# uc-vision/taichi-splatting

Hardware: AMD Instinct MI355X
Metric: fwd+bwd Msplats/s (higher is better)
Workload: dtype f32; 1 GPU; config D: 6000000 random 3D gaussians, 2048x2048, SH deg 3, tile 16, fwd+bwd (render_gaussians, loss=image.sum()); n_gaussians=6000000, tile_size=16, sh_degree=3, mode=single, parallelism=single GPU

## Files before the change

taichi_splatting_amd/csrc/mapper.hip:

```cpp
#pragma clang fp contract(off)
#include "common.h"
#include "frame_internal.h"

namespace ms {

__device__ __forceinline__ void load_point7(const float* __restrict__ points, int64_t i, float g[7]) {
#pragma unroll
  for (int k = 0; k < 7; ++k) g[k] = points[i * 7 + k];
}


__device__ __forceinline__ float readlane_f(float v, int lane) {
  return __int_as_float(__builtin_amdgcn_readlane(__float_as_int(v), lane));
}
__device__ __forceinline__ ObbQuery wave_broadcast(const ObbQuery& q, int lane) {
  ObbQuery r;
  r.inv00 = readlane_f(q.inv00, lane); r.inv01 = readlane_f(q.inv01, lane);
  r.inv10 = readlane_f(q.inv10, lane); r.inv11 = readlane_f(q.inv11, lane);
  r.rel_min_x = readlane_f(q.rel_min_x, lane); r.rel_min_y = readlane_f(q.rel_min_y, lane);
  r.min_tile_x = __builtin_amdgcn_readlane(q.min_tile_x, lane); r.min_tile_y = __builtin_amdgcn_readlane(q.min_tile_y, lane);
  r.span_x = __builtin_amdgcn_readlane(q.span_x, lane); r.span_y = __builtin_amdgcn_readlane(q.span_y, lane);
  return r;
}
__device__ __forceinline__ unsigned long long wide_span_lanes(const ObbQuery& q, bool valid, int* my_span) {
  const int span = valid && q.span_x > 0 && q.span_y > 0 ? q.span_x * q.span_y : 0;
  *my_span = span;
  const int total = (int)readlane_f(wave_sum_to_lane63((float)span), 63);
  int thr = total / 32;
  thr = thr > 16 ? thr : 16;
  return __ballot(span > thr);
}
template <typename F>
__device__ __forceinline__ void wave_walk_span(const ObbQuery& b, int tile_size, int row_begin, int row_end, F on_hits) {
  const int n = b.span_x * b.span_y, lane = lane_id();
  for (int base = 0; base < n; base += 64) {
    const int idx = base + lane;
    bool hit = false;
    int tu = 0, tv = 0;
    if (idx < n) {
      tv = idx / b.span_x; tu = idx - tv * b.span_x;
      const int ty = b.min_tile_y + tv;
      hit = ty >= row_begin && ty < row_end && obb_test_tile(b, tu, tv, tile_size);
    }
    on_hits(hit, b.min_tile_x + tu, b.min_tile_y + tv);
  }
}
__device__ __forceinline__ int count_span(const ObbQuery& q, bool valid, int tile_size, int row_begin, int row_end) {
  int span;
  unsigned long long wide = wide_span_lanes(q, valid, &span);
  const bool mine_is_wide = (wide >> lane_id()) & 1ull;
  int count = 0;
  if (span > 0 && !mine_is_wide) {
    for (int tv = 0; tv < q.span_y; ++tv) {
      const int ty = q.min_tile_y + tv;
      if (ty < row_begin || ty >= row_end) continue;
      for (int tu = 0; tu < q.span_x; ++tu)
        if (obb_test_tile(q, tu, tv, tile_size)) ++count;
    }
  }
  while (wide != 0) {
    const int src = __builtin_ctzll(wide);
    wide &= wide - 1;
    const ObbQuery b = wave_broadcast(q, src);
    int total = 0;
    wave_walk_span(b, tile_size, row_begin, row_end, [&](bool hit, int, int) { total += __builtin_popcountll(__ballot(hit)); });
    if (lane_id() == src) count = total;
  }
  return count;
}
template <typename F>
__device__ __forceinline__ void emit_span(const ObbQuery& q, bool valid, int64_t first, int tile_size, int row_begin,
                                          int row_end, F emit) {
  int span;
  unsigned long long wide = wide_span_lanes(q, valid, &span);
  const bool mine_is_wide = (wide >> lane_id()) & 1ull;
  if (span > 0 && !mine_is_wide) {
    int64_t o = first;
    for (int tu = 0; tu < q.span_x; ++tu) {
      for (int tv = 0; tv < q.span_y; ++tv) {
        const int ty = q.min_tile_y + tv;
        if (ty < row_begin || ty >= row_end) continue;
        if (obb_test_tile(q, tu, tv, tile_size)) emit(o++, q.min_tile_x + tu, ty, -1);
      }
    }
  }
  while (wide != 0) {
    const int src = __builtin_ctzll(wide);
    wide &= wide - 1;
    const ObbQuery b = wave_broadcast(q, src);
    const int lo = __builtin_amdgcn_readlane((int)(uint32_t)first, src), hi = __builtin_amdgcn_readlane((int)(uint32_t)(first >> 32), src);
    int64_t o = (int64_t)(((uint64_t)(uint32_t)hi << 32) | (uint32_t)lo);
    wave_walk_span(b, tile_size, row_begin, row_end, [&](bool hit, int tx, int ty) {
      const unsigned long long m = __ballot(hit);
      if (hit) emit(o + (int)__builtin_amdgcn_mbcnt_hi((uint32_t)(m >> 32), __builtin_amdgcn_mbcnt_lo((uint32_t)m, 0u)), tx, ty, src);
      o += __builtin_popcountll(m);
    });
  }
}

__global__ void __launch_bounds__(256)
tile_count_kernel(const float* __restrict__ points, const int32_t* __restrict__ order,
                  const uint32_t* __restrict__ cull_keys, int64_t v, int image_w,
                  int image_h, int tile_size, float alpha_threshold, int row_begin, int row_end,
                  int32_t* __restrict__ counts, float* __restrict__ ordered_points) {
  const int64_t i = (int64_t)blockIdx.x * blockDim.x + threadIdx.x;
  const bool valid = i < v && !(cull_keys && cull_keys[i] == CULLED_DEPTH_KEY);
  float g[7] = {0.f, 0.f, 1.f, 0.f, 1.f, 1.f, 0.f};
  if (valid) {
    load_point7(points, order ? (int64_t)order[i] : i, g);
    if (ordered_points) {
#pragma unroll
      for (int k = 0; k < 7; ++k) ordered_points[i * 7 + k] = g[k];
    }
  }
  const ObbQuery q = obb_grid_query(g, image_w, image_h, tile_size, alpha_threshold);
  const int count = count_span(q, valid, tile_size, row_begin, row_end);
  if (i < v) counts[i] = count;
}

template <typename KeyT, int MODE>
__global__ void __launch_bounds__(256)
tile_emit_kernel(const float* __restrict__ points, const float* __restrict__ depth,
                 const int32_t* __restrict__ order, const int32_t* __restrict__ cum, int64_t v,
                 int image_w, int image_h, int tile_size, float alpha_threshold, int row_begin,
                 int row_end, int points_ordered, const int32_t* __restrict__ k_limit,
                 KeyT* __restrict__ keys, int32_t* __restrict__ values) {
  const int64_t i = (int64_t)blockIdx.x * blockDim.x + threadIdx.x;
  if (k_limit && *k_limit == 0) return;
  const bool valid = i < v && !(k_limit && cum[i + 1] == cum[i]);
  const int64_t src = valid ? (order ? (int64_t)order[i] : i) : 0;
  float g[7] = {0.f, 0.f, 1.f, 0.f, 1.f, 1.f, 0.f};
  if (valid) load_point7(points, points_ordered ? i : src, g);
  const ObbQuery q = obb_grid_query(g, image_w, image_h, tile_size, alpha_threshold);
  const int tiles_wide = image_w / tile_size;
  KeyT depth_key = 0;
  if (valid) {
    if (MODE == 1) {
      const float c = fminf(fmaxf(depth[src], 0.0f), 1.0f);
      depth_key = (KeyT)(uint32_t)(c * 65535.0f);
    } else if (MODE == 0) {
      depth_key = (KeyT)__float_as_uint(depth[src]);
    }
  }
  const uint32_t dk_lo = (uint32_t)depth_key, dk_hi = (uint32_t)((uint64_t)depth_key >> 32);
  emit_span(q, valid, valid ? (int64_t)cum[i] : 0, tile_size, row_begin, row_end, [&](int64_t o, int tx, int ty, int from) {
    const int64_t tile_id = (int64_t)tx + (int64_t)ty * tiles_wide;
    KeyT dk = depth_key;
    int32_t who = (int32_t)src;
    if (from >= 0) {
      dk = (KeyT)(((uint64_t)(uint32_t)__builtin_amdgcn_readlane((int)dk_hi, from) << 32) | (uint32_t)__builtin_amdgcn_readlane((int)dk_lo, from));
      who = __builtin_amdgcn_readlane((int32_t)src, from);
    }
    if constexpr (MODE == 2) keys[o] = (KeyT)tile_id;
    else if constexpr (MODE == 1) keys[o] = (KeyT)(dk | ((KeyT)tile_id << 16));
    else keys[o] = (KeyT)(dk | ((KeyT)tile_id << 32));
    values[o] = who;
  });
}

template <typename T>
__global__ void __launch_bounds__(256, 8)
tile_count_direct_kernel(const float* __restrict__ points, const T* __restrict__ cull_depth, int64_t v, int image_w,
                         int image_h, int tile_size, float alpha_threshold, int row_begin, int row_end,
                         int32_t* __restrict__ counts) {
  const int64_t i = (int64_t)blockIdx.x * blockDim.x + threadIdx.x;
  const bool valid = i < v && !(cull_depth && !(cull_depth[i] > T(0)));
  float g[7] = {0.f, 0.f, 1.f, 0.f, 1.f, 1.f, 0.f};
  if (valid) load_point7(points, i, g);
  const ObbQuery q = obb_grid_query(g, image_w, image_h, tile_size, alpha_threshold);
  const int count = count_span(q, valid, tile_size, row_begin, row_end);
  if (i < v) counts[i] = count;
}

template <typename T>
__global__ void __launch_bounds__(256)
tile_emit_direct_kernel(const float* __restrict__ points, const T* __restrict__ depth, const int32_t* __restrict__ cum,
                        int64_t v, int image_w, int image_h, int tile_size, float alpha_threshold, int row_begin,
                        int row_end, int depth16, double near_plane, double far_plane,
                        const int32_t* __restrict__ k_limit, uint64_t* __restrict__ keys, int32_t* __restrict__ values) {
  const int64_t i = (int64_t)blockIdx.x * blockDim.x + threadIdx.x;
  if (k_limit && *k_limit == 0) return;
  const int64_t first = i < v ? (int64_t)cum[i] : 0;
  const bool valid = i < v && cum[i + 1] != first;
  float g[7] = {0.f, 0.f, 1.f, 0.f, 1.f, 1.f, 0.f};
  if (valid) load_point7(points, i, g);
  const ObbQuery q = obb_grid_query(g, image_w, image_h, tile_size, alpha_threshold);
  const int tiles_wide = image_w / tile_size;
  const uint32_t depth_key = valid ? (uint32_t)depth_sort_key(depth[i], depth16, near_plane, far_plane) : 0u;
  emit_span(q, valid, first, tile_size, row_begin, row_end, [&](int64_t o, int tx, int ty, int from) {
    const uint64_t tile_id = (uint64_t)((int64_t)tx + (int64_t)ty * tiles_wide);
    uint32_t dk = depth_key;
    int32_t who = (int32_t)i;
    if (from >= 0) { dk = (uint32_t)__builtin_amdgcn_readlane((int)depth_key, from); who = __builtin_amdgcn_readlane((int32_t)i, from); }
    keys[o] = (tile_id << 32) | dk;
    values[o] = who;
  });
}

template <typename T>
__global__ void __launch_bounds__(256)
depth_keys_kernel(const T* __restrict__ depth, int64_t v, int depth16, double near_plane, double far_plane,
                  uint32_t* __restrict__ keys, int32_t* __restrict__ values) {
  const int64_t i = (int64_t)blockIdx.x * blockDim.x + threadIdx.x;
  if (i >= v) return;
  keys[i] = depth_sort_key(depth[i], depth16, near_plane, far_plane);
  values[i] = (int32_t)i;
}

void tile_count_launch(const float* points7, const int32_t* order, const uint32_t* cull_keys, int64_t v, int image_w,
                       int image_h, int tile_size, float alpha_threshold, int row_begin, int row_end,
                       int32_t* out_counts, float* out_ordered, hipStream_t s) {
  tile_count_kernel<<<dim3((unsigned)div_up(v, 256)), dim3(256), 0, s>>>(
      points7, order, cull_keys, v, image_w, image_h, tile_size, alpha_threshold, row_begin, row_end, out_counts, out_ordered);
}

void tile_emit_ordered_launch(const float* ordered_points7, const int32_t* order, const int32_t* cum, int64_t v,
                              int image_w, int image_h, int tile_size, float alpha_threshold, int row_begin,
                              int row_end, const int32_t* k_limit_dev, uint32_t* out_keys, int32_t* out_values,
                              hipStream_t s) {
  tile_emit_kernel<uint32_t, 2><<<dim3((unsigned)div_up(v, 256)), dim3(256), 0, s>>>(
      ordered_points7, nullptr, order, cum, v, image_w, image_h, tile_size, alpha_threshold, row_begin, row_end, 1,
      k_limit_dev, out_keys, out_values);
}

void tile_count_direct_launch(const float* points7, const void* cull_depth, int dtype, int64_t v, int image_w, int image_h,
                              int tile_size, float alpha_threshold, int row_begin, int row_end, int32_t* out_counts,
                              hipStream_t s) {
  const dim3 grid((unsigned)div_up(v, 256)), block(256);
  if (dtype == MS_F64)
    tile_count_direct_kernel<double><<<grid, block, 0, s>>>(points7, (const double*)cull_depth, v, image_w, image_h, tile_size,
                                                            alpha_threshold, row_begin, row_end, out_counts);
  else
    tile_count_direct_kernel<float><<<grid, block, 0, s>>>(points7, (const float*)cull_depth, v, image_w, image_h, tile_size,
                                                           alpha_threshold, row_begin, row_end, out_counts);
}

void tile_emit_direct_launch(const float* points7, const void* depth, int dtype, const int32_t* cum, int64_t v, int image_w,
                             int image_h, int tile_size, float alpha_threshold, int row_begin, int row_end, int depth16,
                             double ndc_near, double ndc_far, const int32_t* k_limit_dev, uint64_t* out_keys,
                             int32_t* out_values, hipStream_t s) {
  const dim3 grid((unsigned)div_up(v, 256)), block(256);
  if (dtype == MS_F64)
    tile_emit_direct_kernel<double><<<grid, block, 0, s>>>(points7, (const double*)depth, cum, v, image_w, image_h, tile_size,
                                                           alpha_threshold, row_begin, row_end, depth16, ndc_near, ndc_far,
                                                           k_limit_dev, out_keys, out_values);
  else
    tile_emit_direct_kernel<float><<<grid, block, 0, s>>>(points7, (const float*)depth, cum, v, image_w, image_h, tile_size,
                                                          alpha_threshold, row_begin, row_end, depth16, ndc_near, ndc_far,
                                                          k_limit_dev, out_keys, out_values);
}

}

using namespace ms;

extern "C" int ms_depth_sort_keys(const void* depth, int64_t v, int depth16, double ndc_near, double ndc_far,
                                  uint32_t* out_keys, int32_t* out_values, int dtype, void* stream) {
  MS_CHECK_ARG(v >= 0, "v < 0");
  MS_CHECK_ARG(dtype == MS_F32 || dtype == MS_F64, "dtype must be MS_F32 or MS_F64");
  if (v == 0) return 0;
  MS_CHECK_ARG(depth && out_keys && out_values, "null pointer");
  const dim3 grid((unsigned)div_up(v, 256)), block(256);
  if (dtype == MS_F32)
    depth_keys_kernel<float><<<grid, block, 0, (hipStream_t)stream>>>((const float*)depth, v, depth16, ndc_near, ndc_far, out_keys, out_values);
  else
    depth_keys_kernel<double><<<grid, block, 0, (hipStream_t)stream>>>((const double*)depth, v, depth16, ndc_near, ndc_far, out_keys, out_values);
  MS_CHECK_LAUNCH();
  return 0;
}

extern "C" int ms_tile_count(const float* points7, const int32_t* order, int64_t v, int image_w, int image_h, int tile_size,
                             float alpha_threshold, int tile_row_begin, int tile_row_end,
                             int32_t* out_counts, float* out_ordered_points7, void* stream) {
  MS_CHECK_ARG(v >= 0, "v < 0");
  MS_CHECK_ARG(tile_size > 0 && image_w > 0 && image_h > 0, "bad image/tile size");
  MS_CHECK_ARG(image_w % tile_size == 0 && image_h % tile_size == 0, "image size must be padded to the tile size");
  if (v == 0) return 0;
  MS_CHECK_ARG(points7 && out_counts, "null pointer");
  tile_count_kernel<<<dim3((unsigned)div_up(v, 256)), dim3(256), 0, (hipStream_t)stream>>>(
      points7, order, nullptr, v, image_w, image_h, tile_size, alpha_threshold, tile_row_begin, tile_row_end, out_counts, out_ordered_points7);
  MS_CHECK_LAUNCH();
  return 0;
}

extern "C" int ms_tile_emit(const float* points7, const float* depth, const int32_t* order, const int32_t* cum,
                            int64_t v, int image_w, int image_h, int tile_size, float alpha_threshold,
                            int tile_row_begin, int tile_row_end, int key_mode, int points_are_ordered,
                            void* out_keys, int32_t* out_values, void* stream) {
  MS_CHECK_ARG(v >= 0, "v < 0");
  MS_CHECK_ARG(key_mode >= 0 && key_mode <= 2, "key_mode must be 0 (tile|depth32), 1 (tile|depth16) or 2 (tile only)");
  MS_CHECK_ARG(tile_size > 0 && image_w > 0 && image_h > 0, "bad image/tile size");
  MS_CHECK_ARG(image_w % tile_size == 0 && image_h % tile_size == 0, "image size must be padded to the tile size");
  if (key_mode == 1) {
    const int64_t tiles = (int64_t)(image_w / tile_size) * (image_h / tile_size);
    MS_CHECK_ARG(tiles <= 65536, "use_depth16 keys hold a 16 bit tile id: too many tiles");
  }
  if (v == 0) return 0;
  MS_CHECK_ARG(points7 && cum && out_keys && out_values, "null pointer");
  MS_CHECK_ARG(key_mode == 2 || depth, "depth is null");
  const dim3 block(256), grid((unsigned)div_up(v, 256));
  hipStream_t s = (hipStream_t)stream;
#define MS_EMIT(KeyT, MODE) tile_emit_kernel<KeyT, MODE><<<grid, block, 0, s>>>(points7, depth, order, cum, v, image_w, image_h, tile_size, alpha_threshold, tile_row_begin, tile_row_end, points_are_ordered, nullptr, (KeyT*)out_keys, out_values)
  if (key_mode == 0) MS_EMIT(uint64_t, 0);
  else if (key_mode == 1) MS_EMIT(uint32_t, 1);
  else MS_EMIT(uint32_t, 2);
#undef MS_EMIT
  MS_CHECK_LAUNCH();
  return 0;
}

extern "C" int ms_tile_emit_keys64(const float* points7, const void* depth, int depth_dtype, const int32_t* cum, int64_t v,
                                   int image_w, int image_h, int tile_size, float alpha_threshold, int tile_row_begin,
                                   int tile_row_end, int depth16, double ndc_near, double ndc_far, uint64_t* out_keys,
                                   int32_t* out_values, void* stream) {
  MS_CHECK_ARG(v >= 0, "v < 0");
  MS_CHECK_ARG(depth_dtype == MS_F32 || depth_dtype == MS_F64, "depth_dtype must be MS_F32 or MS_F64");
  MS_CHECK_ARG(tile_size > 0 && image_w > 0 && image_h > 0, "bad image/tile size");
  MS_CHECK_ARG(image_w % tile_size == 0 && image_h % tile_size == 0, "image size must be padded to the tile size");
  if (depth16) {
    const int64_t tiles = (int64_t)(image_w / tile_size) * (image_h / tile_size);
    MS_CHECK_ARG(tiles <= 65536, "use_depth16 keys hold a 16 bit tile id: too many tiles");
  }
  if (v == 0) return 0;
  MS_CHECK_ARG(points7 && depth && cum && out_keys && out_values, "null pointer");
  tile_emit_direct_launch(points7, depth, depth_dtype, cum, v, image_w, image_h, tile_size, alpha_threshold, tile_row_begin,
                          tile_row_end, depth16, ndc_near > 0.0 ? ndc_near : 0.0, ndc_far, nullptr, out_keys, out_values,
                          (hipStream_t)stream);
  MS_CHECK_LAUNCH();
  return 0;
}
```

taichi_splatting_amd/csrc/scan_sort.hip:

```cpp
#include "common.h"
#include "frame_internal.h"

namespace ms {

constexpr int SCAN_THREADS = 256;
constexpr int SCAN_ITEMS = 16;
constexpr int SCAN_TILE = SCAN_THREADS * SCAN_ITEMS;

__device__ __forceinline__ int block_exclusive_scan(int v, int* lds , int* block_total) {
  const int lane = lane_id(), wave = threadIdx.x >> 6;
  int incl = v;
#pragma unroll
  for (int off = 1; off < 64; off <<= 1) {
    const int t = __shfl_up(incl, off, 64);
    if (lane >= off) incl += t;
  }
  if (lane == 63) lds[wave] = incl;
  __syncthreads();
  int wave_off = 0, total = 0;
#pragma unroll
  for (int w = 0; w < SCAN_THREADS / 64; ++w) {
    const int s = lds[w];
    if (w < wave) wave_off += s;
    total += s;
// ... 70 lines not shown
  int vals[SCAN_ITEMS];
  load_items(in, base, n, vals);
  int s = 0;
#pragma unroll
  for (int k = 0; k < SCAN_ITEMS; ++k) s += vals[k];
  int total;
  int prefix = block_exclusive_scan(s, lds, &total) + block_offsets[blockIdx.x];
#pragma unroll
  for (int k = 0; k < SCAN_ITEMS; ++k) {
    const int v = vals[k];
    vals[k] = prefix;
    prefix += v;
  }
  store_items(out, base, n, vals);
}

constexpr int64_t SCAN_SELF_MAX_BLOCKS = 8192;

__global__ void __launch_bounds__(SCAN_THREADS)
scan_downsweep_self_kernel(const int32_t* __restrict__ in, int64_t n, const int32_t* __restrict__ block_sums,
                           int32_t* __restrict__ out, int32_t* __restrict__ total_host,
                           int32_t* __restrict__ total_copy = nullptr) {
  __shared__ int lds[4];
  int before = 0;
  for (int j = threadIdx.x; j < (int)blockIdx.x; j += SCAN_THREADS) before += block_sums[j];
  int block_prefix;
  block_exclusive_scan(before, lds, &block_prefix);

  const int64_t base = (int64_t)blockIdx.x * SCAN_TILE + (int64_t)threadIdx.x * SCAN_ITEMS;
  int vals[SCAN_ITEMS];
  load_items(in, base, n, vals);
  int s = 0;
#pragma unroll
  for (int k = 0; k < SCAN_ITEMS; ++k) s += vals[k];
  int total;
  int prefix = block_exclusive_scan(s, lds, &total) + block_prefix;
#pragma unroll
  for (int k = 0; k < SCAN_ITEMS; ++k) {
    const int v = vals[k];
    vals[k] = prefix;
    prefix += v;
  }
  store_items(out, base, n, vals);
  if (blockIdx.x == gridDim.x - 1 && threadIdx.x == 0) {
    out[n] = block_prefix + total;
    if (total_copy) *total_copy = block_prefix + total;
    if (total_host) *total_host = block_prefix + total;
  }
}

static size_t scan_tmp_bytes(int64_t n) { return align_up((size_t)div_up(n > 0 ? n : 1, SCAN_TILE) * sizeof(int32_t), 256); }

static int exclusive_scan_i32(const int32_t* in, int64_t n, int32_t* out, int32_t* total_host, void* tmp,
                              hipStream_t s, int32_t* total_copy = nullptr) {
  const int64_t blocks = div_up(n, SCAN_TILE);
  int32_t* block_sums = (int32_t*)tmp;
  scan_block_sums_kernel<<<dim3((unsigned)blocks), dim3(SCAN_THREADS), 0, s>>>(in, n, block_sums);
  if (blocks <= SCAN_SELF_MAX_BLOCKS) {
    scan_downsweep_self_kernel<<<dim3((unsigned)blocks), dim3(SCAN_THREADS), 0, s>>>(in, n, block_sums, out, total_host, total_copy);
    return 0;
  }
  scan_spine_kernel<<<dim3(1), dim3(SCAN_THREADS), 0, s>>>(block_sums, blocks, out + n, total_host, total_copy);
  scan_downsweep_kernel<<<dim3((unsigned)blocks), dim3(SCAN_THREADS), 0, s>>>(in, n, block_sums, out);
  return 0;
}

constexpr int RS_THREADS = 256;
constexpr int RS_WAVES = RS_THREADS / 64;
constexpr int RS_ROUNDS = 16;
constexpr int RS_WAVE_ITEMS = RS_ROUNDS * 64;
constexpr int RS_TILE = RS_THREADS * RS_ROUNDS;
constexpr int RS_RADIX = 256;

template <typename KeyT>
__device__ __forceinline__ unsigned key_digit(KeyT k, int shift, unsigned mask) {
  return (unsigned)(k >> shift) & mask;
}

template <typename KeyT> struct PlainPairs {
  const KeyT* keys;
  const int32_t* vals;
  __device__ __forceinline__ KeyT key(int64_t i) const { return keys[i]; }
  __device__ __forceinline__ int32_t val(int64_t i) const { return vals[i]; }
};
template <typename T> struct DepthPairs {
  const T* depth;
  int depth16;
  double near_plane, far_plane;
  int cull;
  __device__ __forceinline__ uint32_t key(int64_t i) const {
    const T d = depth[i];
    if (cull && !(d > T(0))) return CULLED_DEPTH_KEY;
    return depth_sort_key(d, depth16, near_plane, far_plane);
  }
  __device__ __forceinline__ int32_t val(int64_t i) const { return (int32_t)i; }
};

template <typename KeyT, typename Source, bool VARY = false>
__device__ __forceinline__ void upsweep_block(const Source src, int64_t n, int shift, unsigned mask,
                                              int32_t* __restrict__ hist, int64_t num_blocks,
                                              uint32_t* __restrict__ blk_or = nullptr, uint32_t* __restrict__ blk_and = nullptr) {
  constexpr int RS_COPIES = 4;
  __shared__ unsigned cnt[RS_WAVES][RS_COPIES][RS_RADIX];
  __shared__ unsigned s_or, s_and;
  for (int i = threadIdx.x; i < RS_WAVES * RS_COPIES * RS_RADIX; i += RS_THREADS) (&cnt[0][0][0])[i] = 0;
  if (VARY && threadIdx.x == 0) { s_or = 0u; s_and = ~0u; }
  __syncthreads();
  const int wave = threadIdx.x >> 6, lane = lane_id();
  unsigned* mine = cnt[wave][lane & (RS_COPIES - 1)];
  const int64_t base = (int64_t)blockIdx.x * RS_TILE + (int64_t)wave * RS_WAVE_ITEMS + lane;
  unsigned v_or = 0u, v_and = ~0u;
  if ((int64_t)(blockIdx.x + 1) * RS_TILE <= n) {
    KeyT k[RS_ROUNDS];
#pragma unroll
    for (int j = 0; j < RS_ROUNDS; ++j) k[j] = src.key(base + j * 64);
#pragma unroll
    for (int j = 0; j < RS_ROUNDS; ++j) {
      atomicAdd(&mine[key_digit(k[j], shift, mask)], 1u);
      if (VARY && (uint32_t)k[j] != 0xffffffffu) { v_or |= (uint32_t)k[j]; v_and &= (uint32_t)k[j]; }
    }
  } else {
#pragma unroll 4
    for (int j = 0; j < RS_ROUNDS; ++j) {
      const int64_t i = base + j * 64;
      if (i < n) {
        const KeyT key = src.key(i);
        atomicAdd(&mine[key_digit(key, shift, mask)], 1u);
        if (VARY && (uint32_t)key != 0xffffffffu) { v_or |= (uint32_t)key; v_and &= (uint32_t)key; }
      }
    }
  }
  if (VARY) {
#pragma unroll
    for (int off = 32; off >= 1; off >>= 1) { v_or |= __shfl_xor(v_or, off); v_and &= __shfl_xor(v_and, off); }
    if (lane == 0) { atomicOr(&s_or, v_or); atomicAnd(&s_and, v_and); }
  }
  __syncthreads();
  for (int d = threadIdx.x; d < RS_RADIX; d += RS_THREADS) {
    unsigned t = 0;
#pragma unroll
    for (int w = 0; w < RS_WAVES; ++w)
#pragma unroll
      for (int c = 0; c < RS_COPIES; ++c) t += cnt[w][c][d];
    hist[(int64_t)d * num_blocks + blockIdx.x] = (int32_t)t;
  }
  if (VARY && threadIdx.x == 0) { blk_or[blockIdx.x] = s_or; blk_and[blockIdx.x] = s_and; }
}

template <typename KeyT, typename Source>
__global__ void __launch_bounds__(RS_THREADS)
radix_upsweep_kernel(const Source src, int64_t n, const int32_t* __restrict__ n_dev, int shift, unsigned mask,
                     int32_t* __restrict__ hist, int64_t num_blocks) {
  if (n_dev) n = *n_dev;
  upsweep_block<KeyT, Source>(src, n, shift, mask, hist, num_blocks);
}

__device__ __forceinline__ void row_scan_body(int32_t* __restrict__ hist, int64_t num_blocks, int32_t* __restrict__ digit_totals) {
  __shared__ int lds[4];
  int32_t* row = hist + (int64_t)blockIdx.x * num_blocks;
  int carry = 0;
  for (int64_t base = 0; base < num_blocks; base += SCAN_TILE) {
    const int64_t mine = base + (int64_t)threadIdx.x * SCAN_ITEMS;
    int vals[SCAN_ITEMS];
    load_items(row, mine, num_blocks, vals);
    int s = 0;
#pragma unroll
    for (int k = 0; k < SCAN_ITEMS; ++k) s += vals[k];
    int total;
    int prefix = carry + block_exclusive_scan(s, lds, &total);
#pragma unroll
    for (int k = 0; k < SCAN_ITEMS; ++k) {
      const int v = vals[k];
      vals[k] = prefix;
      prefix += v;
    }
    store_items(row, mine, num_blocks, vals);
    carry += total;
  }
  if (threadIdx.x == 0) digit_totals[blockIdx.x] = carry;
}

__global__ void __launch_bounds__(SCAN_THREADS)
radix_row_scan_kernel(int32_t* __restrict__ hist, int64_t num_blocks, int32_t* __restrict__ digit_totals) {
  row_scan_body(hist, num_blocks, digit_totals);
}

template <typename KeyT> struct DownsweepShared {
  unsigned cnt[RS_WAVES][RS_RADIX];
  int scan[4];
  unsigned digit_shift[RS_RADIX];
  KeyT keys[RS_TILE];
  int32_t vals[RS_TILE];
};

template <typename KeyT, bool FULL, typename Source>
__device__ __forceinline__ void downsweep_block(DownsweepShared<KeyT>& sh, const Source src, KeyT* __restrict__ keys_out,
                                                int32_t* __restrict__ vals_out, int64_t n, int shift, unsigned mask,
                                                const int32_t* __restrict__ hist_scanned,
                                                const int32_t* __restrict__ digit_totals, int64_t num_blocks) {
  for (int i = threadIdx.x; i < RS_WAVES * RS_RADIX; i += RS_THREADS) (&sh.cnt[0][0])[i] = 0;
  __syncthreads();

  const int wave = threadIdx.x >> 6, lane = lane_id();
  const int64_t base = (int64_t)blockIdx.x * RS_TILE + (int64_t)wave * RS_WAVE_ITEMS + lane;
  const unsigned long long lanes_below = (1ull << lane) - 1ull;

  KeyT k[RS_ROUNDS];
  int32_t v[RS_ROUNDS];
  unsigned rank[RS_ROUNDS];

#pragma unroll
  for (int j = 0; j < RS_ROUNDS; ++j) {
    const int64_t i = base + j * 64;
    const bool valid = FULL || i < n;
    k[j] = valid ? src.key(i) : (KeyT)0;
    v[j] = valid ? src.val(i) : 0;
  }

#pragma unroll
  for (int j = 0; j < RS_ROUNDS; ++j) {
    const int64_t i = base + j * 64;
    const bool valid = FULL || i < n;
    const unsigned d = key_digit(k[j], shift, mask);
    const unsigned long long valid_lanes = FULL ? ~0ull : __ballot(valid);
    unsigned peers_lo = (unsigned)valid_lanes, peers_hi = (unsigned)(valid_lanes >> 32);
#pragma unroll
    for (int b = 0; b < 8; ++b) {
      const int m = __builtin_amdgcn_sbfe((int)d, b, 1);
      const unsigned long long bal = __ballot(m != 0);
      peers_lo &= ~((unsigned)bal ^ (unsigned)m);
      peers_hi &= ~((unsigned)(bal >> 32) ^ (unsigned)m);
    }
    const unsigned long long peers = ((unsigned long long)peers_hi << 32) | peers_lo;
    const unsigned below = (unsigned)__popcll(peers & lanes_below);
    unsigned prev = 0;
    if (valid) {
      prev = sh.cnt[wave][d];
    }
    __builtin_amdgcn_wave_barrier();
    if (valid && below == 0) sh.cnt[wave][d] = prev + (unsigned)__popcll(peers);
    __builtin_amdgcn_wave_barrier();
    rank[j] = prev + below;
  }
  __syncthreads();

  {
    const int d = threadIdx.x;
    unsigned total = 0;
#pragma unroll
    for (int w = 0; w < RS_WAVES; ++w) total += sh.cnt[w][d];
    int block_total;
    const unsigned local = (unsigned)block_exclusive_scan((int)total, sh.scan, &block_total);
    unsigned run = local;
#pragma unroll
    for (int w = 0; w < RS_WAVES; ++w) {
      const unsigned c = sh.cnt[w][d];
      sh.cnt[w][d] = run;
      run += c;
    }
    int all_items;
    const unsigned digit_base = (unsigned)block_exclusive_scan(digit_totals[d], sh.scan, &all_items);
    sh.digit_shift[d] = digit_base + (unsigned)hist_scanned[(int64_t)d * num_blocks + blockIdx.x] - local;
  }
  __syncthreads();

#pragma unroll
  for (int j = 0; j < RS_ROUNDS; ++j) {
    const int64_t i = base + j * 64;
    if (FULL || i < n) {
      const unsigned d = key_digit(k[j], shift, mask);
      const unsigned lp = sh.cnt[wave][d] + rank[j];
      sh.keys[lp] = k[j];
      sh.vals[lp] = v[j];
    }
  }
  __syncthreads();
  const int64_t block_base = (int64_t)blockIdx.x * RS_TILE;
  const int block_items = FULL ? RS_TILE : (int)(n - block_base);
#pragma unroll
  for (int j = 0; j < RS_ROUNDS; ++j) {
    const int idx = (int)threadIdx.x + j * RS_THREADS;
    if (FULL || idx < block_items) {
      const KeyT key = sh.keys[idx];
      const unsigned d = key_digit(key, shift, mask);
      const int64_t pos = (int64_t)(unsigned)(sh.digit_shift[d] + (unsigned)idx);
      keys_out[pos] = key;
      vals_out[pos] = sh.vals[idx];
    }
  }
}

template <typename KeyT, typename Source>
__global__ void __launch_bounds__(RS_THREADS)
radix_downsweep_kernel(const Source src,
                       KeyT* __restrict__ keys_out, int32_t* __restrict__ vals_out, int64_t n,
                       const int32_t* __restrict__ n_dev, int shift,
                       unsigned mask, const int32_t* __restrict__ hist_scanned,
                       const int32_t* __restrict__ digit_totals, int64_t num_blocks) {
  __shared__ DownsweepShared<KeyT> sh;
  if (n_dev) {
    n = *n_dev;
    if ((int64_t)blockIdx.x * RS_TILE >= n) return;
  }
  if ((int64_t)(blockIdx.x + 1) * RS_TILE <= n)
    downsweep_block<KeyT, true>(sh, src, keys_out, vals_out, n, shift, mask, hist_scanned, digit_totals, num_blocks);
  else
    downsweep_block<KeyT, false>(sh, src, keys_out, vals_out, n, shift, mask, hist_scanned, digit_totals, num_blocks);
}

template <typename KeyT>
__global__ void __launch_bounds__(256)
copy_pairs_kernel(const KeyT* __restrict__ ki, const int32_t* __restrict__ vi, KeyT* __restrict__ ko,
                  int32_t* __restrict__ vo, int64_t n) {
  const int64_t i = (int64_t)blockIdx.x * blockDim.x + threadIdx.x;
  if (i < n) { ko[i] = ki[i]; vo[i] = vi[i]; }
}

struct SortTmp {
  size_t hist_off, scan_off, keys_off, vals_off, keys2_off, vals2_off, vary_off, total;
};

static SortTmp sort_tmp_layout(int64_t n, int key_bytes, bool adaptive = false) {
  const int64_t blocks = div_up(n > 0 ? n : 1, RS_TILE);
  SortTmp t;
  size_t off = 0;
  t.hist_off = off; off += align_up((size_t)(RS_RADIX * blocks + 1) * sizeof(int32_t), 256);
  t.scan_off = off; off += align_up((size_t)RS_RADIX * sizeof(int32_t), 256);
  t.keys_off = off; off += align_up((size_t)n * key_bytes, 256);
  t.vals_off = off; off += align_up((size_t)n * sizeof(int32_t), 256);
  t.keys2_off = t.vals2_off = t.vary_off = off;
  if (adaptive) {
    t.keys2_off = off; off += align_up((size_t)n * key_bytes, 256);
    t.vals2_off = off; off += align_up((size_t)n * sizeof(int32_t), 256);
    t.vary_off = off; off += align_up((size_t)(64 + 2 * blocks) * sizeof(uint32_t), 256);
  }
  t.total = off;
  return t;
}

template <typename KeyT, typename First>
static int radix_sort_passes(const First first, KeyT* keys_out, int32_t* vals_out, int64_t n, int begin_bit, int end_bit,
                             char* tmp, hipStream_t s, const int32_t* n_dev = nullptr) {
  const int64_t blocks = div_up(n, RS_TILE);
  const SortTmp lay = sort_tmp_layout(n, sizeof(KeyT));
  int32_t* hist = (int32_t*)(tmp + lay.hist_off);
  int32_t* digit_totals = (int32_t*)(tmp + lay.scan_off);
  KeyT* keys_alt = (KeyT*)(tmp + lay.keys_off);
  int32_t* vals_alt = (int32_t*)(tmp + lay.vals_off);
  const int passes = (end_bit - begin_bit + 7) / 8;
  const dim3 grid((unsigned)blocks), block(RS_THREADS);
  PlainPairs<KeyT> src{nullptr, nullptr};
  const int total_bits = end_bit - begin_bit, base_bits = total_bits / passes, wide = total_bits % passes;
  int shift = begin_bit;
  for (int p = 0; p < passes; shift += base_bits + (p < wide ? 1 : 0), ++p) {
    const int bits = base_bits + (p < wide ? 1 : 0);
    const unsigned mask = (1u << bits) - 1u;
    const bool to_out = ((passes - 1 - p) % 2) == 0;
    KeyT* dst_k = to_out ? keys_out : keys_alt;
    int32_t* dst_v = to_out ? vals_out : vals_alt;
    if (p == 0) radix_upsweep_kernel<KeyT, First><<<grid, block, 0, s>>>(first, n, n_dev, shift, mask, hist, blocks);
    else radix_upsweep_kernel<KeyT, PlainPairs<KeyT>><<<grid, block, 0, s>>>(src, n, n_dev, shift, mask, hist, blocks);
    radix_row_scan_kernel<<<dim3(RS_RADIX), dim3(SCAN_THREADS), 0, s>>>(hist, blocks, digit_totals);
    if (p == 0) radix_downsweep_kernel<KeyT, First><<<grid, block, 0, s>>>(first, dst_k, dst_v, n, n_dev, shift, mask, hist, digit_totals, blocks);
    else radix_downsweep_kernel<KeyT, PlainPairs<KeyT>><<<grid, block, 0, s>>>(src, dst_k, dst_v, n, n_dev, shift, mask, hist, digit_totals, blocks);
    src = PlainPairs<KeyT>{dst_k, dst_v};
  }
  return 0;
}

struct AdaptiveBufs {
  uint32_t *k_alt[2], *k_out;
  int32_t *v_alt[2], *v_out;
  uint32_t* vary;
};

__device__ __forceinline__ void adaptive_route(uint32_t vary, int p, int passes, bool& active, int& k, bool& last) {
// ... 335 lines not shown
```

taichi_splatting_amd/csrc/splat_math.h:

```cpp
#pragma once

#if defined(__HIPCC__)
#include <hip/hip_runtime.h>
#define MS_HD __host__ __device__ __forceinline__
#else
#include <cmath>
#define MS_HD inline
#endif

namespace ms {

template <typename T> MS_HD T t_min(T a, T b) { return a < b ? a : b; }
template <typename T> MS_HD T t_max(T a, T b) { return a > b ? a : b; }
template <typename T> MS_HD T t_clamp(T x, T lo, T hi) { return t_min(t_max(x, lo), hi); }
MS_HD float t_sqrt(float x) { return sqrtf(x); }
MS_HD double t_sqrt(double x) { return sqrt(x); }
MS_HD float t_exp(float x) { return expf(x); }
MS_HD double t_exp(double x) { return exp(x); }
MS_HD float t_log(float x) { return logf(x); }
MS_HD double t_log(double x) { return log(x); }
MS_HD float t_abs(float x) { return fabsf(x); }
MS_HD double t_abs(double x) { return fabs(x); }
MS_HD float t_floor(float x) { return floorf(x); }
MS_HD double t_floor(double x) { return floor(x); }
// ... 293 lines not shown
}

template <typename T>
MS_HD T gaussian_pdf_with_grad(T px, T py, const T* g, T dmean[2], T daxis[2], T dsigma[2]) {
  const T dx = px - g[0], dy = py - g[1];
  const T ax = g[2], ay = g[3], sx = g[4], sy = g[5];
  const T tx = (dx * ax + dy * ay) / sx;
  const T ty = (dx * -ay + dy * ax) / sy;
  const T tx2 = tx * tx, ty2 = ty * ty;
  const T p = t_exp(T(-0.5) * (tx2 + ty2));
  dsigma[0] = tx2 * p / sx;
  dsigma[1] = ty2 * p / sy;
  const T tx_s = tx / sx, ty_s = ty / sy;
  daxis[0] = p * (tx_s * -dx + ty_s * -dy);
  daxis[1] = p * (tx_s * -dy + ty_s * dx);
  dmean[0] = p * (tx_s * ax + ty_s * -ay);
  dmean[1] = p * (tx_s * ay + ty_s * ax);
  return p;
}

template <typename T>
MS_HD T s_sig(T x, T sigma) {
  const T z = x / sigma;
  return T(1) / (T(1) + t_exp(T(-1.6) * z - T(0.07) * z * z * z));
}

template <typename T>
MS_HD T gaussian_pdf_antialias(T px, T py, const T* g) {
  const T dx = px - g[0], dy = py - g[1];
  const T sx = g[4], sy = g[5];
  const T tx = dx * g[2] + dy * g[3];
  const T ty = dx * -g[3] + dy * g[2];
  const T Sx1 = s_sig(tx + T(0.5), sx), Sx2 = s_sig(tx - T(0.5), sx);
  const T Sy1 = s_sig(ty + T(0.5), sy), Sy2 = s_sig(ty - T(0.5), sy);
  return T(2 * 3.14159265358979323846) * sx * (Sx1 - Sx2) * sy * (Sy1 - Sy2);
}

template <typename T>
MS_HD void s_sig_grad(T x, T sigma, T& s, T& ds_dx, T& ds_dsigma) {
  const T z = x / sigma;
  s = T(1) / (T(1) + t_exp(T(-1.6) * z - T(0.07) * z * z * z));
  const T ds = (T(1.6) + T(0.21) * z * z) * s * (T(1) - s);
  ds_dx = ds / sigma;
  ds_dsigma = ds_dx * -z;
}

template <typename T>
MS_HD T gaussian_pdf_antialias_with_grad(T px, T py, const T* g, T dmean[2], T daxis[2], T dsigma[2]) {
  const T dx = px - g[0], dy = py - g[1];
  const T ax = g[2], ay = g[3], sx = g[4], sy = g[5];
  const T tx = dx * ax + dy * ay;
  const T ty = dx * -ay + dy * ax;

  T Sx1, dSx1, dSx1s, Sx2, dSx2, dSx2s, Sy1, dSy1, dSy1s, Sy2, dSy2, dSy2s;
  s_sig_grad(tx + T(0.5), sx, Sx1, dSx1, dSx1s);
  s_sig_grad(tx - T(0.5), sx, Sx2, dSx2, dSx2s);
  s_sig_grad(ty + T(0.5), sy, Sy1, dSy1, dSy1s);
  s_sig_grad(ty - T(0.5), sy, Sy2, dSy2, dSy2s);

  const T ix = sx * (Sx1 - Sx2);
  const T iy = sy * (Sy1 - Sy2);
  const T tau = T(2 * 3.14159265358979323846);
  const T i2d = tau * ix * iy;

  const T dSx = iy * sx * (dSx1 - dSx2);
  const T dSy = ix * sy * (dSy1 - dSy2);

  dmean[0] = tau * (dSx * -ax + dSy * ay);
  dmean[1] = tau * (dSx * -ay + dSy * -ax);
  dsigma[0] = tau * iy * (Sx1 - Sx2 + (dSx1s - dSx2s) * sx);
  dsigma[1] = tau * ix * (Sy1 - Sy2 + (dSy1s - dSy2s) * sy);
  daxis[0] = tau * (dSx * dx + dSy * dy);
  daxis[1] = tau * (dSx * dy + dSy * -dx);
  return i2d;
}

struct ObbQuery {
  float inv00, inv01, inv10, inv11;
  float rel_min_x, rel_min_y;
  int min_tile_x, min_tile_y;
  int span_x, span_y;
};

MS_HD ObbQuery obb_grid_query(const float* g , int image_w, int image_h, int tile_size,
                              float alpha_threshold) {
  const float mx = g[0], my = g[1], ax = g[2], ay = g[3], sgx = g[4], sgy = g[5], alpha = g[6];
  const float gs = sqrtf(2.0f * logf(alpha / alpha_threshold));
  const float sx = sgx * gs, sy = sgy * gs;
  const float a2x = -ay, a2y = ax;

  const float v1x = ax * sx, v1y = ay * sx, v2x = a2x * sy, v2y = a2y * sy;
  const float ex = sqrtf(v1x * v1x + v2x * v2x), ey = sqrtf(v1y * v1y + v2y * v2y);
  const float min_x = mx - ex, min_y = my - ey, max_x = mx + ex, max_y = my + ey;

  ObbQuery q;
  q.inv00 = ax / sx; q.inv01 = ay / sx;
  q.inv10 = a2x / sy; q.inv11 = a2y / sy;

  const float ts = (float)tile_size;
  const int max_tile_x = (image_w - 1) / tile_size, max_tile_y = (image_h - 1) / tile_size;
  int lo_x = (min_x == min_x) ? (int)floorf(min_x / ts) : 0x3fffffff;
  int lo_y = (min_y == min_y) ? (int)floorf(min_y / ts) : 0x3fffffff;
  lo_x = lo_x > 0 ? lo_x : 0;
  lo_y = lo_y > 0 ? lo_y : 0;
  int hi_x = (max_x == max_x) ? (int)ceilf(max_x / ts) : 0;
  int hi_y = (max_y == max_y) ? (int)ceilf(max_y / ts) : 0;
  hi_x = hi_x > lo_x + 1 ? hi_x : lo_x + 1;
  hi_y = hi_y > lo_y + 1 ? hi_y : lo_y + 1;
  hi_x = hi_x < max_tile_x + 1 ? hi_x : max_tile_x + 1;
  hi_y = hi_y < max_tile_y + 1 ? hi_y : max_tile_y + 1;

  q.min_tile_x = lo_x; q.min_tile_y = lo_y;
  q.span_x = hi_x - lo_x; q.span_y = hi_y - lo_y;
  q.rel_min_x = (float)(lo_x * tile_size) - mx;
  q.rel_min_y = (float)(lo_y * tile_size) - my;
  return q;
}

MS_HD bool obb_test_tile(const ObbQuery& q, int u, int v, int tile_size) {
  const float lx = q.rel_min_x + (float)(u * tile_size), ly = q.rel_min_y + (float)(v * tile_size);
  const float ux = lx + (float)tile_size, uy = ly + (float)tile_size;
  bool separates = false;
  {
    const float p0 = q.inv00 * lx + q.inv01 * ly, p1 = q.inv00 * ux + q.inv01 * ly;
    const float p2 = q.inv00 * ux + q.inv01 * uy, p3 = q.inv00 * lx + q.inv01 * uy;
    const float mn = fminf(fminf(p0, p1), fminf(p2, p3)), mxv = fmaxf(fmaxf(p0, p1), fmaxf(p2, p3));
    if (mn > 1.0f || mxv < -1.0f) separates = true;
  }
  {
    const float p0 = q.inv10 * lx + q.inv11 * ly, p1 = q.inv10 * ux + q.inv11 * ly;
    const float p2 = q.inv10 * ux + q.inv11 * uy, p3 = q.inv10 * lx + q.inv11 * uy;
    const float mn = fminf(fminf(p0, p1), fminf(p2, p3)), mxv = fmaxf(fmaxf(p0, p1), fmaxf(p2, p3));
    if (mn > 1.0f || mxv < -1.0f) separates = true;
  }
  return !separates;
}

}
```

Before: 2033 Msplats/s.

## Use reciprocal tile scaling, two-phase value scatter in radix downsweep, early point loads

Result: no change. 2029 Msplats/s (-0.2%).

```diff
diff --git a/taichi_splatting_amd/csrc/mapper.hip b/taichi_splatting_amd/csrc/mapper.hip
--- a/taichi_splatting_amd/csrc/mapper.hip
+++ b/taichi_splatting_amd/csrc/mapper.hip
@@ -101,7 +101,7 @@
 __global__ void __launch_bounds__(256)
 tile_count_kernel(const float* __restrict__ points, const int32_t* __restrict__ order,
                   const uint32_t* __restrict__ cull_keys, int64_t v, int image_w,
-                  int image_h, int tile_size, float alpha_threshold, int row_begin, int row_end,
+                  int image_h, int tile_size, float alpha_threshold, float inv_tile, int row_begin, int row_end,
                   int32_t* __restrict__ counts, float* __restrict__ ordered_points) {
   const int64_t i = (int64_t)blockIdx.x * blockDim.x + threadIdx.x;
   const bool valid = i < v && !(cull_keys && cull_keys[i] == CULLED_DEPTH_KEY);
@@ -113,7 +113,7 @@
       for (int k = 0; k < 7; ++k) ordered_points[i * 7 + k] = g[k];
     }
   }
-  const ObbQuery q = obb_grid_query(g, image_w, image_h, tile_size, alpha_threshold);
+  const ObbQuery q = obb_grid_query(g, image_w, image_h, tile_size, alpha_threshold, inv_tile);
   const int count = count_span(q, valid, tile_size, row_begin, row_end);
   if (i < v) counts[i] = count;
 }
@@ -122,7 +122,7 @@
 __global__ void __launch_bounds__(256)
 tile_emit_kernel(const float* __restrict__ points, const float* __restrict__ depth,
                  const int32_t* __restrict__ order, const int32_t* __restrict__ cum, int64_t v,
-                 int image_w, int image_h, int tile_size, float alpha_threshold, int row_begin,
+                 int image_w, int image_h, int tile_size, float alpha_threshold, float inv_tile, int row_begin,
                  int row_end, int points_ordered, const int32_t* __restrict__ k_limit,
                  KeyT* __restrict__ keys, int32_t* __restrict__ values) {
   const int64_t i = (int64_t)blockIdx.x * blockDim.x + threadIdx.x;
@@ -131,7 +131,7 @@
   const int64_t src = valid ? (order ? (int64_t)order[i] : i) : 0;
   float g[7] = {0.f, 0.f, 1.f, 0.f, 1.f, 1.f, 0.f};
   if (valid) load_point7(points, points_ordered ? i : src, g);
-  const ObbQuery q = obb_grid_query(g, image_w, image_h, tile_size, alpha_threshold);
+  const ObbQuery q = obb_grid_query(g, image_w, image_h, tile_size, alpha_threshold, inv_tile);
   const int tiles_wide = image_w / tile_size;
   KeyT depth_key = 0;
   if (valid) {
@@ -161,13 +161,13 @@
 template <typename T>
 __global__ void __launch_bounds__(256, 8)
 tile_count_direct_kernel(const float* __restrict__ points, const T* __restrict__ cull_depth, int64_t v, int image_w,
-                         int image_h, int tile_size, float alpha_threshold, int row_begin, int row_end,
+                         int image_h, int tile_size, float alpha_threshold, float inv_tile, int row_begin, int row_end,
                          int32_t* __restrict__ counts) {
   const int64_t i = (int64_t)blockIdx.x * blockDim.x + threadIdx.x;
+  float g[7] = {0.f, 0.f, 1.f, 0.f, 1.f, 1.f, 0.f};
+  if (i < v) load_point7(points, i, g);
   const bool valid = i < v && !(cull_depth && !(cull_depth[i] > T(0)));
-  float g[7] = {0.f, 0.f, 1.f, 0.f, 1.f, 1.f, 0.f};
-  if (valid) load_point7(points, i, g);
-  const ObbQuery q = obb_grid_query(g, image_w, image_h, tile_size, alpha_threshold);
+  const ObbQuery q = obb_grid_query(g, image_w, image_h, tile_size, alpha_threshold, inv_tile);
   const int count = count_span(q, valid, tile_size, row_begin, row_end);
   if (i < v) counts[i] = count;
 }
@@ -175,8 +175,8 @@
 template <typename T>
 __global__ void __launch_bounds__(256)
 tile_emit_direct_kernel(const float* __restrict__ points, const T* __restrict__ depth, const int32_t* __restrict__ cum,
-                        int64_t v, int image_w, int image_h, int tile_size, float alpha_threshold, int row_begin,
-                        int row_end, int depth16, double near_plane, double far_plane,
+                        int64_t v, int image_w, int image_h, int tile_size, float alpha_threshold, float inv_tile,
+                        int row_begin, int row_end, int depth16, double near_plane, double far_plane,
                         const int32_t* __restrict__ k_limit, uint64_t* __restrict__ keys, int32_t* __restrict__ values) {
   const int64_t i = (int64_t)blockIdx.x * blockDim.x + threadIdx.x;
   if (k_limit && *k_limit == 0) return;
@@ -184,7 +184,7 @@
   const bool valid = i < v && cum[i + 1] != first;
   float g[7] = {0.f, 0.f, 1.f, 0.f, 1.f, 1.f, 0.f};
   if (valid) load_point7(points, i, g);
-  const ObbQuery q = obb_grid_query(g, image_w, image_h, tile_size, alpha_threshold);
+  const ObbQuery q = obb_grid_query(g, image_w, image_h, tile_size, alpha_threshold, inv_tile);
   const int tiles_wide = image_w / tile_size;
   const uint32_t depth_key = valid ? (uint32_t)depth_sort_key(depth[i], depth16, near_plane, far_plane) : 0u;
   emit_span(q, valid, first, tile_size, row_begin, row_end, [&](int64_t o, int tx, int ty, int from) {
@@ -211,7 +211,8 @@
                        int image_h, int tile_size, float alpha_threshold, int row_begin, int row_end,
                        int32_t* out_counts, float* out_ordered, hipStream_t s) {
   tile_count_kernel<<<dim3((unsigned)div_up(v, 256)), dim3(256), 0, s>>>(
-      points7, order, cull_keys, v, image_w, image_h, tile_size, alpha_threshold, row_begin, row_end, out_counts, out_ordered);
+      points7, order, cull_keys, v, image_w, image_h, tile_size, alpha_threshold, exact_inv_tile(tile_size), row_begin, row_end, out_counts,
+      out_ordered);
 }
 
 void tile_emit_ordered_launch(const float* ordered_points7, const int32_t* order, const int32_t* cum, int64_t v,
@@ -219,7 +220,7 @@
                               int row_end, const int32_t* k_limit_dev, uint32_t* out_keys, int32_t* out_values,
                               hipStream_t s) {
   tile_emit_kernel<uint32_t, 2><<<dim3((unsigned)div_up(v, 256)), dim3(256), 0, s>>>(
-      ordered_points7, nullptr, order, cum, v, image_w, image_h, tile_size, alpha_threshold, row_begin, row_end, 1,
+      ordered_points7, nullptr, order, cum, v, image_w, image_h, tile_size, alpha_threshold, exact_inv_tile(tile_size), row_begin, row_end, 1,
       k_limit_dev, out_keys, out_values);
 }
 
@@ -229,10 +230,10 @@
   const dim3 grid((unsigned)div_up(v, 256)), block(256);
   if (dtype == MS_F64)
     tile_count_direct_kernel<double><<<grid, block, 0, s>>>(points7, (const double*)cull_depth, v, image_w, image_h, tile_size,
-                                                            alpha_threshold, row_begin, row_end, out_counts);
+                                                            alpha_threshold, exact_inv_tile(tile_size), row_begin, row_end, out_counts);
   else
     tile_count_direct_kernel<float><<<grid, block, 0, s>>>(points7, (const float*)cull_depth, v, image_w, image_h, tile_size,
-                                                           alpha_threshold, row_begin, row_end, out_counts);
+                                                           alpha_threshold, exact_inv_tile(tile_size), row_begin, row_end, out_counts);
 }
 
 void tile_emit_direct_launch(const float* points7, const void* depth, int dtype, const int32_t* cum, int64_t v, int image_w,
@@ -242,11 +243,11 @@
   const dim3 grid((unsigned)div_up(v, 256)), block(256);
   if (dtype == MS_F64)
     tile_emit_direct_kernel<double><<<grid, block, 0, s>>>(points7, (const double*)depth, cum, v, image_w, image_h, tile_size,
-                                                           alpha_threshold, row_begin, row_end, depth16, ndc_near, ndc_far,
+                                                           alpha_threshold, exact_inv_tile(tile_size), row_begin, row_end, depth16, ndc_near, ndc_far,
                                                            k_limit_dev, out_keys, out_values);
   else
     tile_emit_direct_kernel<float><<<grid, block, 0, s>>>(points7, (const float*)depth, cum, v, image_w, image_h, tile_size,
-                                                          alpha_threshold, row_begin, row_end, depth16, ndc_near, ndc_far,
+                                                          alpha_threshold, exact_inv_tile(tile_size), row_begin, row_end, depth16, ndc_near, ndc_far,
                                                           k_limit_dev, out_keys, out_values);
 }
 
@@ -278,7 +279,8 @@
   if (v == 0) return 0;
   MS_CHECK_ARG(points7 && out_counts, "null pointer");
   tile_count_kernel<<<dim3((unsigned)div_up(v, 256)), dim3(256), 0, (hipStream_t)stream>>>(
-      points7, order, nullptr, v, image_w, image_h, tile_size, alpha_threshold, tile_row_begin, tile_row_end, out_counts, out_ordered_points7);
+      points7, order, nullptr, v, image_w, image_h, tile_size, alpha_threshold, exact_inv_tile(tile_size), tile_row_begin, tile_row_end, out_counts,
+      out_ordered_points7);
   MS_CHECK_LAUNCH();
   return 0;
 }
@@ -300,7 +302,7 @@
   MS_CHECK_ARG(key_mode == 2 || depth, "depth is null");
   const dim3 block(256), grid((unsigned)div_up(v, 256));
   hipStream_t s = (hipStream_t)stream;
-#define MS_EMIT(KeyT, MODE) tile_emit_kernel<KeyT, MODE><<<grid, block, 0, s>>>(points7, depth, order, cum, v, image_w, image_h, tile_size, alpha_threshold, tile_row_begin, tile_row_end, points_are_ordered, nullptr, (KeyT*)out_keys, out_values)
+#define MS_EMIT(KeyT, MODE) tile_emit_kernel<KeyT, MODE><<<grid, block, 0, s>>>(points7, depth, order, cum, v, image_w, image_h, tile_size, alpha_threshold, exact_inv_tile(tile_size), tile_row_begin, tile_row_end, points_are_ordered, nullptr, (KeyT*)out_keys, out_values)
   if (key_mode == 0) MS_EMIT(uint64_t, 0);
   else if (key_mode == 1) MS_EMIT(uint32_t, 1);
   else MS_EMIT(uint32_t, 2);
diff --git a/taichi_splatting_amd/csrc/scan_sort.hip b/taichi_splatting_amd/csrc/scan_sort.hip
--- a/taichi_splatting_amd/csrc/scan_sort.hip
+++ b/taichi_splatting_amd/csrc/scan_sort.hip
@@ -176,6 +176,8 @@
   const int32_t* vals;
   __device__ __forceinline__ KeyT key(int64_t i) const { return keys[i]; }
   __device__ __forceinline__ int32_t val(int64_t i) const { return vals[i]; }
+  __device__ __forceinline__ KeyT key(int64_t first, unsigned off) const { return (keys + first)[off]; }
+  __device__ __forceinline__ int32_t val(int64_t first, unsigned off) const { return (vals + first)[off]; }
 };
 template <typename T> struct DepthPairs {
   const T* depth;
@@ -188,6 +190,8 @@
     return depth_sort_key(d, depth16, near_plane, far_plane);
   }
   __device__ __forceinline__ int32_t val(int64_t i) const { return (int32_t)i; }
+  __device__ __forceinline__ uint32_t key(int64_t first, unsigned off) const { return key(first + off); }
+  __device__ __forceinline__ int32_t val(int64_t first, unsigned off) const { return val(first + off); }
 };
 
 template <typename KeyT, typename Source, bool VARY = false>
@@ -280,11 +284,12 @@
 }
 
 template <typename KeyT> struct DownsweepShared {
+  static constexpr bool TWO_PHASE = sizeof(KeyT) == 8;
   unsigned cnt[RS_WAVES][RS_RADIX];
   int scan[4];
   unsigned digit_shift[RS_RADIX];
   KeyT keys[RS_TILE];
-  int32_t vals[RS_TILE];
+  int32_t vals[TWO_PHASE ? 1 : RS_TILE];
 };
 
 template <typename KeyT, bool FULL, typename Source>
@@ -296,9 +301,11 @@
   __syncthreads();
 
   const int wave = threadIdx.x >> 6, lane = lane_id();
-  const int64_t base = (int64_t)blockIdx.x * RS_TILE + (int64_t)wave * RS_WAVE_ITEMS + lane;
+  const int64_t block_first = (int64_t)blockIdx.x * RS_TILE;
+  const int64_t base = block_first + (int64_t)wave * RS_WAVE_ITEMS + lane;
   const unsigned long long lanes_below = (1ull << lane) - 1ull;
 
+  constexpr bool TWO_PHASE = DownsweepShared<KeyT>::TWO_PHASE;
   KeyT k[RS_ROUNDS];
   int32_t v[RS_ROUNDS];
   unsigned rank[RS_ROUNDS];
@@ -307,8 +314,9 @@
   for (int j = 0; j < RS_ROUNDS; ++j) {
     const int64_t i = base + j * 64;
     const bool valid = FULL || i < n;
-    k[j] = valid ? src.key(i) : (KeyT)0;
-    v[j] = valid ? src.val(i) : 0;
+    const unsigned off = (unsigned)(wave * RS_WAVE_ITEMS + lane + j * 64);
+    k[j] = valid ? src.key(block_first, off) : (KeyT)0;
+    if (!TWO_PHASE) v[j] = valid ? src.val(block_first, off) : 0;
   }
 
 #pragma unroll
@@ -358,6 +366,14 @@
   }
   __syncthreads();
 
+  int32_t* const lds_vals = TWO_PHASE ? reinterpret_cast<int32_t*>(sh.keys) : sh.vals;
+  if (TWO_PHASE) {
+#pragma unroll
+    for (int j = 0; j < RS_ROUNDS; ++j) {
+      const unsigned off = (unsigned)(wave * RS_WAVE_ITEMS + lane + j * 64);
+      v[j] = (FULL || base + j * 64 < n) ? src.val(block_first, off) : 0;
+    }
+  }
 #pragma unroll
   for (int j = 0; j < RS_ROUNDS; ++j) {
     const int64_t i = base + j * 64;
@@ -365,27 +381,43 @@
       const unsigned d = key_digit(k[j], shift, mask);
       const unsigned lp = sh.cnt[wave][d] + rank[j];
       sh.keys[lp] = k[j];
-      sh.vals[lp] = v[j];
+      if (TWO_PHASE) rank[j] = lp;
+      else lds_vals[lp] = v[j];
     }
   }
   __syncthreads();
   const int64_t block_base = (int64_t)blockIdx.x * RS_TILE;
   const int block_items = FULL ? RS_TILE : (int)(n - block_base);
+  unsigned pos[RS_ROUNDS];
 #pragma unroll
   for (int j = 0; j < RS_ROUNDS; ++j) {
     const int idx = (int)threadIdx.x + j * RS_THREADS;
     if (FULL || idx < block_items) {
       const KeyT key = sh.keys[idx];
       const unsigned d = key_digit(key, shift, mask);
-      const int64_t pos = (int64_t)(unsigned)(sh.digit_shift[d] + (unsigned)idx);
-      keys_out[pos] = key;
-      vals_out[pos] = sh.vals[idx];
+      pos[j] = sh.digit_shift[d] + (unsigned)idx;
+      keys_out[(int64_t)pos[j]] = key;
+      if (!TWO_PHASE) vals_out[(int64_t)pos[j]] = lds_vals[idx];
+    }
+  }
+  if (TWO_PHASE) {
+    __syncthreads();
+#pragma unroll
+    for (int j = 0; j < RS_ROUNDS; ++j) {
+      const int64_t i = base + j * 64;
+      if (FULL || i < n) lds_vals[rank[j]] = v[j];
+    }
+    __syncthreads();
+#pragma unroll
+    for (int j = 0; j < RS_ROUNDS; ++j) {
+      const int idx = (int)threadIdx.x + j * RS_THREADS;
+      if (FULL || idx < block_items) vals_out[(int64_t)pos[j]] = lds_vals[idx];
     }
   }
 }
 
 template <typename KeyT, typename Source>
-__global__ void __launch_bounds__(RS_THREADS)
+__global__ void __launch_bounds__(RS_THREADS, 4)
 radix_downsweep_kernel(const Source src,
                        KeyT* __restrict__ keys_out, int32_t* __restrict__ vals_out, int64_t n,
                        const int32_t* __restrict__ n_dev, int shift,
diff --git a/taichi_splatting_amd/csrc/splat_math.h b/taichi_splatting_amd/csrc/splat_math.h
--- a/taichi_splatting_amd/csrc/splat_math.h
+++ b/taichi_splatting_amd/csrc/splat_math.h
@@ -399,8 +399,12 @@
   int span_x, span_y;
 };
 
+inline float exact_inv_tile(int tile_size) {
+  return tile_size > 0 && (tile_size & (tile_size - 1)) == 0 ? 1.0f / (float)tile_size : 0.0f;
+}
+
 MS_HD ObbQuery obb_grid_query(const float* g , int image_w, int image_h, int tile_size,
-                              float alpha_threshold) {
+                              float alpha_threshold, float inv_tile = 0.0f) {
   const float mx = g[0], my = g[1], ax = g[2], ay = g[3], sgx = g[4], sgy = g[5], alpha = g[6];
   const float gs = sqrtf(2.0f * logf(alpha / alpha_threshold));
   const float sx = sgx * gs, sy = sgy * gs;
@@ -416,12 +420,18 @@
 
   const float ts = (float)tile_size;
   const int max_tile_x = (image_w - 1) / tile_size, max_tile_y = (image_h - 1) / tile_size;
-  int lo_x = (min_x == min_x) ? (int)floorf(min_x / ts) : 0x3fffffff;
-  int lo_y = (min_y == min_y) ? (int)floorf(min_y / ts) : 0x3fffffff;
+  float tmin_x, tmin_y, tmax_x, tmax_y;
+  if (inv_tile != 0.0f) {
+    tmin_x = min_x * inv_tile; tmin_y = min_y * inv_tile; tmax_x = max_x * inv_tile; tmax_y = max_y * inv_tile;
+  } else {
+    tmin_x = min_x / ts; tmin_y = min_y / ts; tmax_x = max_x / ts; tmax_y = max_y / ts;
+  }
+  int lo_x = (min_x == min_x) ? (int)floorf(tmin_x) : 0x3fffffff;
+  int lo_y = (min_y == min_y) ? (int)floorf(tmin_y) : 0x3fffffff;
   lo_x = lo_x > 0 ? lo_x : 0;
   lo_y = lo_y > 0 ? lo_y : 0;
-  int hi_x = (max_x == max_x) ? (int)ceilf(max_x / ts) : 0;
-  int hi_y = (max_y == max_y) ? (int)ceilf(max_y / ts) : 0;
+  int hi_x = (max_x == max_x) ? (int)ceilf(tmax_x) : 0;
+  int hi_y = (max_y == max_y) ? (int)ceilf(tmax_y) : 0;
   hi_x = hi_x > lo_x + 1 ? hi_x : lo_x + 1;
   hi_y = hi_y > lo_y + 1 ? hi_y : lo_y + 1;
   hi_x = hi_x < max_tile_x + 1 ? hi_x : max_tile_x + 1;
```
